# hkust-vgd/nerfstyle

Measured on AMD Instinct MI355X. Metric: train Mrays/sec, higher is better.
Workload: dtype f16

## Files before the change

nerfstyle_amd/csrc/table_scatter.hip:

```cpp
#include "field_common.h"
#include "lattice.h"
#include "table_scatter.h"


__device__ __forceinline__ bool seq_nonzero(const float4 &v) {
    return ((__float_as_uint(v.x) | __float_as_uint(v.y) | __float_as_uint(v.z) | __float_as_uint(v.w)) << 1) != 0u;
}

constexpr int TS_THREADS = 256;
constexpr int LAT_MAX_SLOTS = (int)(((65536 - 16 * sizeof(NsrLevel)) / (TS_THREADS / 64) - 256) / 16 / 64 * 64);
struct LatState {
    uint32_t b0, b1, b2;
};

template <int S>
__device__ __forceinline__ void lat_flush_level(float4 *__restrict__ lat4, uint32_t *__restrict__ rows, uint32_t b0, uint32_t b1, uint32_t b2,
                                                const NsrLevel &lv, float *__restrict__ gt, int lane, bool td, bool tc, uint32_t xl) {
    constexpr int NC = S * S * S;
    constexpr int RS = (16 / S) * S;
    const int t = lane >> 2, i = lane & 3;
    const int g = lane >> 4, j = lane & 15;
    const bool on = (i < 2) ? td : tc;
    const float *lf = reinterpret_cast<const float *>(lat4);
#pragma unroll 1
    for (int k0 = 0; k0 < NC; k0 += 4 * RS) {
        const int k = k0 + g * RS + j;
        float4 v = make_float4(0.f, 0.f, 0.f, 0.f);
        if (j < RS && k < NC) v = lat4[k];
        const bool nz = seq_nonzero(v);
        if (__ballot(nz) == 0ull) continue;
        bool out = false;
        if (nz) {
            constexpr uint32_t MZ = (65536u + S * S - 1u) / (S * S), MY = (65536u + S - 1u) / S;
            const uint32_t z = __umul24((uint32_t)k, MZ) >> 16, r = (uint32_t)k - __umul24(z, (uint32_t)(S * S));
            const uint32_t y = __umul24(r, MY) >> 16, x = r - __umul24(y, (uint32_t)S);
            out = x < xl;
            if (out) rows[lane] = lv.offset + lat_row(lv, b0 + x, b1 + y, b2 + z);
        }
        const unsigned long long m = __ballot(out);
        __builtin_amdgcn_wave_barrier();
#pragma unroll
        for (int q = 0; q < 4; q++) {
            if (k0 + RS * q >= NC) break;
            if (((m >> (16 * q)) & 0xFFFFull) == 0ull) continue;
            const bool rec = (m >> (16 * q + t)) & 1ull;
            if (rec) {
                const float val = lf[(k0 + RS * q + t) * 4 + i];
                const uint32_t row = rows[16 * q + t];
                if (on) atomicAdd(gt + (size_t)row * 4 + i, val);
            }
        }
        __builtin_amdgcn_wave_barrier();
        if (nz) lat4[k] = make_float4(0.f, 0.f, 0.f, 0.f);
        __builtin_amdgcn_wave_barrier();
        if (nz && !out) lat4[k - (int)xl] = v;
    }
}

__device__ __forceinline__ void lat_flush_dispatch(float4 *__restrict__ lat, int fl, const LatState &st, uint32_t xl_lane,
                                                   const NsrLevel *__restrict__ lds_lv, float *__restrict__ gt, int lane, bool td, bool tc) {
    const uint32_t o0 = (uint32_t)__builtin_amdgcn_readlane((int)st.b0, fl * 4);
    if (o0 == LAT_NONE) return;
    const uint32_t o1 = (uint32_t)__builtin_amdgcn_readlane((int)st.b1, fl * 4);
    const uint32_t o2 = (uint32_t)__builtin_amdgcn_readlane((int)st.b2, fl * 4);
    const uint32_t xl = (uint32_t)__builtin_amdgcn_readlane((int)xl_lane, fl * 4);
    const NsrLevel flv = lds_lv[fl];
    float4 *lf = lat + (flv.pad_ >> 8);
    uint32_t *rows = reinterpret_cast<uint32_t *>(lat) - 64;
    switch (flv.pad_ & 0xFu) {
    case 3: lat_flush_level<3>(lf, rows, o0, o1, o2, flv, gt, lane, td, tc, xl); break;
    case 4: lat_flush_level<4>(lf, rows, o0, o1, o2, flv, gt, lane, td, tc, xl); break;
    case 5: lat_flush_level<5>(lf, rows, o0, o1, o2, flv, gt, lane, td, tc, xl); break;
    default: lat_flush_level<6>(lf, rows, o0, o1, o2, flv, gt, lane, td, tc, xl); break;
    }
}


struct TableScatterArgs {
    const float *xyzs;
    const uint32_t *perm;
    const int32_t *m_dev;
    uint32_t M;
    const float4 *gin;
    float *grad_tables;
    float bmin[3], bsize[3];
    int td, tc;
    uint32_t lat_slots;
    NsrLevel lv[16];
};

constexpr int TS_RING = 8;
static size_t ts_wave_bytes(uint32_t lat_slots) { return 256 + (size_t)lat_slots * 16; }

__global__ void __launch_bounds__(TS_THREADS)
k_table_scatter(TableScatterArgs a) {
    extern __shared__ __attribute__((aligned(16))) char smem[];
    NsrLevel *lds_lv = reinterpret_cast<NsrLevel *>(smem);
    if (threadIdx.x < 16) lds_lv[threadIdx.x] = a.lv[threadIdx.x];
    const int lane = threadIdx.x & 63, wave = threadIdx.x >> 6;
    char *base = smem + 16 * sizeof(NsrLevel) + (size_t)wave * (256 + (size_t)a.lat_slots * 16);
    float4 *lat = reinterpret_cast<float4 *>(base + 256);
    for (uint32_t k = lane; k < a.lat_slots; k += 64) lat[k] = make_float4(0.f, 0.f, 0.f, 0.f);
    __syncthreads();

    const uint32_t Mc = FIELD_COUNT(a);
    if (Mc == 0) return;
    const uint32_t ntiles = (Mc + 15) / 16;
    const uint32_t nwaves = gridDim.x * (TS_THREADS / 64), gw = blockIdx.x * (TS_THREADS / 64) + wave;
    const uint32_t per = (ntiles + nwaves - 1) / nwaves;
    const uint32_t w_begin = min(gw * per, ntiles), w_end = min(w_begin + per, ntiles);
    if (w_begin >= w_end) return;
    const int s = lane & 15;
    const int l = lane >> 2, py = lane & 1, pz = (lane >> 1) & 1;
    const NsrLevel lv = lds_lv[l];
    const uint32_t S = lv.pad_ & 0xFu, ashift = (lv.pad_ >> 4) & 0xFu;
    float4 *const mylat = lat + (lv.pad_ >> 8) + ((uint32_t)pz * S + (uint32_t)py) * S;
    const bool td = a.td != 0, tc = a.tc != 0;
    float *const gt = a.grad_tables;
    const float kq = (float)(1 << LAT_KEY_BITS), rk = 1.0f / kq;
    LatState st;
    st.b0 = st.b1 = st.b2 = LAT_NONE;
    uint32_t cur_key = LAT_NONE;
    float bf0 = 0.f, bf1 = 0.f, bf2 = 0.f;
    const float lscale = (float)lv.resolution;
    const float lcmax = (float)(lv.resolution - 1u);
    const float Sf = (float)S, Sm2 = (float)(S - 2u);
    const float sy = py ? 1.0f : -1.0f, oy = py ? 0.0f : 1.0f, sz = pz ? 1.0f : -1.0f, oz = pz ? 0.0f : 1.0f;

    auto fetch_idx = [&](uint32_t tile) -> uint32_t { return a.perm[min(tile * 16 + (uint32_t)s, Mc - 1u)]; };
    uint32_t idx = fetch_idx(w_begin);
    uint32_t idx_next = w_begin + 1 < w_end ? fetch_idx(w_begin + 1) : idx;
    float x0 = a.xyzs[(size_t)idx * 3], x1 = a.xyzs[(size_t)idx * 3 + 1], x2 = a.xyzs[(size_t)idx * 3 + 2];
    auto ts_gin = [&](uint32_t v, int ln) { return a.gin[(size_t)(uint32_t)__builtin_amdgcn_readlane((int)v, ln) * 16 + l]; };
    float4 gq[TS_RING];
#pragma unroll
    for (int i = 0; i < TS_RING; i++) gq[i] = ts_gin(idx, i);

    for (uint32_t tile = w_begin; tile < w_end; tile++) {
        float nx0 = x0, nx1 = x1, nx2 = x2;
        uint32_t idx_nn = idx_next;
        if (tile + 1 < w_end) {
            nx0 = a.xyzs[(size_t)idx_next * 3]; nx1 = a.xyzs[(size_t)idx_next * 3 + 1]; nx2 = a.xyzs[(size_t)idx_next * 3 + 2];
            if (tile + 2 < w_end) idx_nn = fetch_idx(tile + 2);
        }
        const bool valid = tile * 16 + (uint32_t)s < Mc;
        const float u0 = field_unit(x0, a.bmin[0], a.bsize[0]), u1 = field_unit(x1, a.bmin[1], a.bsize[1]),
                    u2 = field_unit(x2, a.bmin[2], a.bsize[2]);
        const bool live = valid && field_in_unit_cube(u0, u1, u2);
        const uint32_t live16 = (uint32_t)(__ballot(live) & 0xFFFFull);
        const uint32_t q0 = (uint32_t)fminf(fmaxf(u0 * kq, 0.0f), kq - 1.0f), q1 = (uint32_t)fminf(fmaxf(u1 * kq, 0.0f), kq - 1.0f),
                       q2 = (uint32_t)fminf(fmaxf(u2 * kq, 0.0f), kq - 1.0f);
        const uint32_t bkey = q0 | (q1 << LAT_KEY_BITS) | (q2 << (2 * LAT_KEY_BITS));
        const uint32_t bkey_e = live ? bkey : LAT_NONE;
        const uint32_t bkey_l = (uint32_t)__builtin_amdgcn_update_dpp((int)cur_key, (int)bkey_e, 0x111, 0xF, 0xF, false);
        const uint32_t chg16 = (uint32_t)(__ballot(bkey_e != bkey_l) & 0xFFFFull);
#pragma unroll 1
        for (int part = 0; part < 16 / TS_RING; part++) {
            const bool wrap = part == 16 / TS_RING - 1;
            const uint32_t src = wrap ? idx_next : idx;
            const int src_lane0 = wrap ? 0 : (part + 1) * TS_RING;
#pragma unroll
            for (int ri = 0; ri < TS_RING; ri++) {
                const int step = part * TS_RING + ri;
                const float4 gr = gq[ri];
                if ((live16 >> step) & 1u) {
                    uint32_t key = cur_key;
                    if ((chg16 >> step) & 1u) key = (uint32_t)__builtin_amdgcn_readlane((int)bkey, step);
                    if (key != cur_key) {
                        cur_key = key;
                        const uint32_t kq0 = key & ((1u << LAT_KEY_BITS) - 1u), kq1 = (key >> LAT_KEY_BITS) & ((1u << LAT_KEY_BITS) - 1u),
                                       kq2 = key >> (2 * LAT_KEY_BITS);
                        const float o0 = (float)((kq0 >> ashift) << ashift) * rk, o1 = (float)((kq1 >> ashift) << ashift) * rk,
                                    o2 = (float)((kq2 >> ashift) << ashift) * rk;
                        float ff;
                        uint32_t n0, n1, n2;
                        nsr_grid_locate(o0, lv.resolution, 1, ff, n0);
                        nsr_grid_locate(o1, lv.resolution, 1, ff, n1);
                        nsr_grid_locate(o2, lv.resolution, 1, ff, n2);
                        const bool chg = (n0 != st.b0) | (n1 != st.b1) | (n2 != st.b2);
                        const uint32_t dx = n0 - st.b0;
                        const bool carry = (st.b0 != LAT_NONE) & (n1 == st.b1) & (n2 == st.b2) & (dx - 1u < S - 1u);
                        const uint32_t xl = carry ? dx : S;
                        unsigned long long mm = __ballot(chg);
                        while (mm) {
                            const int fl = (int)(__builtin_ctzll(mm) >> 2);
                            mm &= ~(0xFull << (fl * 4));
                            lat_flush_dispatch(lat, fl, st, xl, lds_lv, gt, lane, td, tc);
                        }
                        if (chg) { st.b0 = n0; st.b1 = n1; st.b2 = n2; bf0 = (float)n0; bf1 = (float)n1; bf2 = (float)n2; }
                    }
                    const float su0 = __builtin_bit_cast(float, __builtin_amdgcn_readlane(__builtin_bit_cast(int, u0), step));
                    const float su1 = __builtin_bit_cast(float, __builtin_amdgcn_readlane(__builtin_bit_cast(int, u1), step));
                    const float su2 = __builtin_bit_cast(float, __builtin_amdgcn_readlane(__builtin_bit_cast(int, u2), step));
                    float f0, f1, f2, cf0, cf1, cf2;
                    {
#pragma clang fp contract(off)
                        const float p0 = su0 * lscale, p1 = su1 * lscale, p2 = su2 * lscale;
                        cf0 = fminf(floorf(p0), lcmax); cf1 = fminf(floorf(p1), lcmax); cf2 = fminf(floorf(p2), lcmax);
                        f0 = p0 - cf0; f1 = p1 - cf1; f2 = p2 - cf2;
                    }
                    const float d0 = cf0 - bf0, d1 = cf1 - bf1, d2 = cf2 - bf2;
                    const float r0 = fminf(d0, Sm2), r1 = fminf(d1, Sm2), r2 = fminf(d2, Sm2);
                    const float wyz = fmaf(f1, sy, oy) * fmaf(f2, sz, oz);
                    float wB = f0 * wyz, wA = wyz - wB;
                    if (fmaxf(d0, fmaxf(d1, d2)) > Sm2) {
                        const uint32_t c0 = (uint32_t)cf0, c1 = (uint32_t)cf1, c2 = (uint32_t)cf2;
                        const uint32_t rowA = lv.offset + lat_row(lv, c0, c1 + (uint32_t)py, c2 + (uint32_t)pz);
                        const uint32_t rowB = lv.offset + lat_row(lv, c0 + 1u, c1 + (uint32_t)py, c2 + (uint32_t)pz);
                        const float ga[4] = {gr.x, gr.y, gr.z, gr.w};
#pragma unroll
                        for (int i = 0; i < 4; i++) {
                            if ((i < 2 ? td : tc) && ga[i] != 0.0f) {
                                atomicAdd(gt + (size_t)rowA * 4 + i, wA * ga[i]);
                                atomicAdd(gt + (size_t)rowB * 4 + i, wB * ga[i]);
                            }
                        }
                        wA = 0.0f;
                        wB = 0.0f;
                    }
                    float4 *const slot = mylat + (uint32_t)fmaf(fmaf(r2, Sf, r1), Sf, r0);
                    float4 va = slot[0], vb = slot[1];
                    va.x = fmaf(wA, gr.x, va.x); va.y = fmaf(wA, gr.y, va.y); va.z = fmaf(wA, gr.z, va.z); va.w = fmaf(wA, gr.w, va.w);
                    vb.x = fmaf(wB, gr.x, vb.x); vb.y = fmaf(wB, gr.y, vb.y); vb.z = fmaf(wB, gr.z, vb.z); vb.w = fmaf(wB, gr.w, vb.w);
                    slot[0] = va;
                    slot[1] = vb;
                }
                asm volatile("" ::: "memory");
                gq[ri] = ts_gin(src, src_lane0 + ri);
            }
        }
        x0 = nx0; x1 = nx1; x2 = nx2;
        idx = idx_next;
        idx_next = idx_nn;
    }
    __builtin_amdgcn_wave_barrier();
#pragma unroll 1
    for (int fl = 0; fl < 16; fl++) lat_flush_dispatch(lat, fl, st, S, lds_lv, gt, lane, td, tc);
}

bool nsr_table_scatter_supported(const NsrLevel *lv) {
    LatGeom g;
    return lat_geometry(lv, g, (uint32_t)LAT_MAX_SLOTS);
}

int nsr_table_scatter_launch(const NsrLevel *levels, const float *bmin, const float *bsize, const float *xyzs, const uint32_t *perm,
                             const int32_t *m_dev, uint32_t M, const void *gin, float *grad_tables, int td, int tc, hipStream_t s) {
    TableScatterArgs a;
    LatGeom g;
    if (!lat_geometry(levels, g, (uint32_t)LAT_MAX_SLOTS)) return NSR_ERR_UNSUPPORTED;
    uint32_t total = 0;
    for (int l = 0; l < 16; l++) {
        a.lv[l] = levels[l];
        a.lv[l].pad_ = (uint32_t)g.S[l] | ((uint32_t)g.shift[l] << 4) | ((uint32_t)g.base[l] << 8);
        total = g.base[l] + (uint32_t)g.S[l] * g.S[l] * g.S[l];
    }
    a.lat_slots = (total + 63u) & ~63u;
    a.xyzs = xyzs; a.perm = perm; a.m_dev = m_dev; a.M = M; a.gin = (const float4 *)gin; a.grad_tables = grad_tables;
    for (int i = 0; i < 3; i++) { a.bmin[i] = bmin[i]; a.bsize[i] = bsize[i]; }
    a.td = td; a.tc = tc;
    const size_t lds = 16 * sizeof(NsrLevel) + (TS_THREADS / 64) * ts_wave_bytes(a.lat_slots);
    if (lds > 65536) return NSR_ERR_UNSUPPORTED;
    uint32_t nblocks = 256u * 16u;
    const uint32_t ntiles = (M + 15) / 16;
    if (nblocks > (ntiles + 3) / 4) nblocks = (ntiles + 3) / 4;
    if (nblocks == 0) nblocks = 1;
    return nsr_launch_lds<k_table_scatter>(65536, dim3(nblocks), dim3(TS_THREADS), lds, s, a);
}
```

Measured before the change: 23.51.

## Batch per-sample cell locate across quads and broadcast via DPP

Rather than every lane redundantly computing floor and fraction and slot index for each broadcast sample step, the kernel now computes these for four steps at once. It gathers the four samples' coordinates into lane quads with ds_bpermute and later fetches each step's values through quad DPP moves. The locate is redone when the lattice base moves, and out-of-range samples take a recomputed global-atomic path driven by a ballot mask. This cuts repeated scalar-broadcast ALU work per step but adds bpermute/DPP traffic, extra ballots and register pressure.

```diff
diff --git a/nerfstyle_amd/csrc/table_scatter.hip b/nerfstyle_amd/csrc/table_scatter.hip
--- a/nerfstyle_amd/csrc/table_scatter.hip
+++ b/nerfstyle_amd/csrc/table_scatter.hip
@@ -90,6 +90,24 @@
 };
 
 constexpr int TS_RING = 8;
+static_assert(TS_RING % 4 == 0, "a quad of steps (one locate pass) must not straddle two parts of the ring");
+
+template <int K>
+__device__ __forceinline__ int quad_lane(int v) {
+    return __builtin_amdgcn_update_dpp(0, v, K * 0x55, 0xF, 0xF, true);
+}
+__device__ __forceinline__ int quad_lane_i(int v, int k) {
+    switch (k & 3) {
+    case 0: return quad_lane<0>(v);
+    case 1: return quad_lane<1>(v);
+    case 2: return quad_lane<2>(v);
+    default: return quad_lane<3>(v);
+    }
+}
+__device__ __forceinline__ float quad_lane_f(float v, int k) {
+    return __builtin_bit_cast(float, quad_lane_i(__builtin_bit_cast(int, v), k));
+}
+
 static size_t ts_wave_bytes(uint32_t lat_slots) { return 256 + (size_t)lat_slots * 16; }
 
 __global__ void __launch_bounds__(TS_THREADS)
@@ -136,6 +154,30 @@
 #pragma unroll
     for (int i = 0; i < TS_RING; i++) gq[i] = ts_gin(idx, i);
 
+    float rq_f0 = 0.f, rq_f1 = 0.f, rq_f2 = 0.f;
+    uint32_t rq_slot = 0u;
+    unsigned long long rq_past = 0ull;
+    float us0 = 0.f, us1 = 0.f, us2 = 0.f;
+    const int rq_lane4 = (lane & 3) * 4;
+    auto locate_quad = [&](int q) {
+        const int from = q * 16 + rq_lane4;
+        const float su0 = __builtin_bit_cast(float, __builtin_amdgcn_ds_bpermute(from, __builtin_bit_cast(int, us0)));
+        const float su1 = __builtin_bit_cast(float, __builtin_amdgcn_ds_bpermute(from, __builtin_bit_cast(int, us1)));
+        const float su2 = __builtin_bit_cast(float, __builtin_amdgcn_ds_bpermute(from, __builtin_bit_cast(int, us2)));
+        float cf0, cf1, cf2;
+        {
+#pragma clang fp contract(off)
+            const float p0 = su0 * lscale, p1 = su1 * lscale, p2 = su2 * lscale;
+            cf0 = fminf(floorf(p0), lcmax); cf1 = fminf(floorf(p1), lcmax); cf2 = fminf(floorf(p2), lcmax);
+            rq_f0 = p0 - cf0; rq_f1 = p1 - cf1; rq_f2 = p2 - cf2;
+        }
+        const float d0 = cf0 - bf0, d1 = cf1 - bf1, d2 = cf2 - bf2;
+        const float r0 = __builtin_amdgcn_fmed3f(d0, 0.0f, Sm2), r1 = __builtin_amdgcn_fmed3f(d1, 0.0f, Sm2),
+                    r2 = __builtin_amdgcn_fmed3f(d2, 0.0f, Sm2);
+        rq_slot = (uint32_t)fmaf(fmaf(r2, Sf, r1), Sf, r0);
+        rq_past = __ballot(fmaxf(d0, fmaxf(d1, d2)) > Sm2);
+    };
+
     for (uint32_t tile = w_begin; tile < w_end; tile++) {
         float nx0 = x0, nx1 = x1, nx2 = x2;
         uint32_t idx_nn = idx_next;
@@ -148,6 +190,7 @@
                     u2 = field_unit(x2, a.bmin[2], a.bsize[2]);
         const bool live = valid && field_in_unit_cube(u0, u1, u2);
         const uint32_t live16 = (uint32_t)(__ballot(live) & 0xFFFFull);
+        us0 = live ? u0 : 0.0f; us1 = live ? u1 : 0.0f; us2 = live ? u2 : 0.0f;
         const uint32_t q0 = (uint32_t)fminf(fmaxf(u0 * kq, 0.0f), kq - 1.0f), q1 = (uint32_t)fminf(fmaxf(u1 * kq, 0.0f), kq - 1.0f),
                        q2 = (uint32_t)fminf(fmaxf(u2 * kq, 0.0f), kq - 1.0f);
         const uint32_t bkey = q0 | (q1 << LAT_KEY_BITS) | (q2 << (2 * LAT_KEY_BITS));
@@ -163,6 +206,7 @@
             for (int ri = 0; ri < TS_RING; ri++) {
                 const int step = part * TS_RING + ri;
                 const float4 gr = gq[ri];
+                if ((ri & 3) == 0 && ((live16 >> step) & 0xFu)) locate_quad(step >> 2);
                 if ((live16 >> step) & 1u) {
                     uint32_t key = cur_key;
                     if ((chg16 >> step) & 1u) key = (uint32_t)__builtin_amdgcn_readlane((int)bkey, step);
@@ -188,37 +232,39 @@
                             lat_flush_dispatch(lat, fl, st, xl, lds_lv, gt, lane, td, tc);
                         }
                         if (chg) { st.b0 = n0; st.b1 = n1; st.b2 = n2; bf0 = (float)n0; bf1 = (float)n1; bf2 = (float)n2; }
+                        if (__ballot(chg)) locate_quad(step >> 2);
                     }
-                    const float su0 = __builtin_bit_cast(float, __builtin_amdgcn_readlane(__builtin_bit_cast(int, u0), step));
-                    const float su1 = __builtin_bit_cast(float, __builtin_amdgcn_readlane(__builtin_bit_cast(int, u1), step));
-                    const float su2 = __builtin_bit_cast(float, __builtin_amdgcn_readlane(__builtin_bit_cast(int, u2), step));
-                    float f0, f1, f2, cf0, cf1, cf2;
-                    {
-#pragma clang fp contract(off)
-                        const float p0 = su0 * lscale, p1 = su1 * lscale, p2 = su2 * lscale;
-                        cf0 = fminf(floorf(p0), lcmax); cf1 = fminf(floorf(p1), lcmax); cf2 = fminf(floorf(p2), lcmax);
-                        f0 = p0 - cf0; f1 = p1 - cf1; f2 = p2 - cf2;
-                    }
-                    const float d0 = cf0 - bf0, d1 = cf1 - bf1, d2 = cf2 - bf2;
-                    const float r0 = fminf(d0, Sm2), r1 = fminf(d1, Sm2), r2 = fminf(d2, Sm2);
+                    const float f0 = quad_lane_f(rq_f0, ri), f1 = quad_lane_f(rq_f1, ri), f2 = quad_lane_f(rq_f2, ri);
+                    const uint32_t rslot = (uint32_t)quad_lane_i((int)rq_slot, ri);
                     const float wyz = fmaf(f1, sy, oy) * fmaf(f2, sz, oz);
                     float wB = f0 * wyz, wA = wyz - wB;
-                    if (fmaxf(d0, fmaxf(d1, d2)) > Sm2) {
-                        const uint32_t c0 = (uint32_t)cf0, c1 = (uint32_t)cf1, c2 = (uint32_t)cf2;
-                        const uint32_t rowA = lv.offset + lat_row(lv, c0, c1 + (uint32_t)py, c2 + (uint32_t)pz);
-                        const uint32_t rowB = lv.offset + lat_row(lv, c0 + 1u, c1 + (uint32_t)py, c2 + (uint32_t)pz);
-                        const float ga[4] = {gr.x, gr.y, gr.z, gr.w};
+                    if (rq_past & (0x1111111111111111ull << (ri & 3))) {
+                        const float su0 = __builtin_bit_cast(float, __builtin_amdgcn_readlane(__builtin_bit_cast(int, us0), step));
+                        const float su1 = __builtin_bit_cast(float, __builtin_amdgcn_readlane(__builtin_bit_cast(int, us1), step));
+                        const float su2 = __builtin_bit_cast(float, __builtin_amdgcn_readlane(__builtin_bit_cast(int, us2), step));
+                        float cf0, cf1, cf2;
+                        {
+#pragma clang fp contract(off)
+                            cf0 = fminf(floorf(su0 * lscale), lcmax); cf1 = fminf(floorf(su1 * lscale), lcmax);
+                            cf2 = fminf(floorf(su2 * lscale), lcmax);
+                        }
+                        if ((rq_past >> ((lane & ~3) | (ri & 3))) & 1ull) {
+                            const uint32_t c0 = (uint32_t)cf0, c1 = (uint32_t)cf1, c2 = (uint32_t)cf2;
+                            const uint32_t rowA = lv.offset + lat_row(lv, c0, c1 + (uint32_t)py, c2 + (uint32_t)pz);
+                            const uint32_t rowB = lv.offset + lat_row(lv, c0 + 1u, c1 + (uint32_t)py, c2 + (uint32_t)pz);
+                            const float ga[4] = {gr.x, gr.y, gr.z, gr.w};
 #pragma unroll
-                        for (int i = 0; i < 4; i++) {
-                            if ((i < 2 ? td : tc) && ga[i] != 0.0f) {
-                                atomicAdd(gt + (size_t)rowA * 4 + i, wA * ga[i]);
-                                atomicAdd(gt + (size_t)rowB * 4 + i, wB * ga[i]);
+                            for (int i = 0; i < 4; i++) {
+                                if ((i < 2 ? td : tc) && ga[i] != 0.0f) {
+                                    atomicAdd(gt + (size_t)rowA * 4 + i, wA * ga[i]);
+                                    atomicAdd(gt + (size_t)rowB * 4 + i, wB * ga[i]);
+                                }
                             }
+                            wA = 0.0f;
+                            wB = 0.0f;
                         }
-                        wA = 0.0f;
-                        wB = 0.0f;
                     }
-                    float4 *const slot = mylat + (uint32_t)fmaf(fmaf(r2, Sf, r1), Sf, r0);
+                    float4 *const slot = mylat + rslot;
                     float4 va = slot[0], vb = slot[1];
                     va.x = fmaf(wA, gr.x, va.x); va.y = fmaf(wA, gr.y, va.y); va.z = fmaf(wA, gr.z, va.z); va.w = fmaf(wA, gr.w, va.w);
                     vb.x = fmaf(wB, gr.x, vb.x); vb.y = fmaf(wB, gr.y, vb.y); vb.z = fmaf(wB, gr.z, vb.z); vb.w = fmaf(wB, gr.w, vb.w);
```

Result: faster. 23.82, median of 6 (+1.3%).
